# FAST-ASR/MarkovModels.jl

Measured on AMD Instinct MI355X. Metric: pdfposteriors_frames_per_sec, higher is better.
Workload: dtype f32

## Files before the change

markovmodels.jl_amd/csrc/mm_engine.hip:

```cpp
#include <hip/hip_runtime.h>
#include <dlfcn.h>

#include <algorithm>
#include <atomic>
#include <cmath>
#include <cstdio>
#include <cstdlib>
#include <chrono>
#include <cstring>
#include <limits>
#include <new>
#include <map>
#include <memory>
#include <mutex>
#include <string>
#include <thread>
#include <vector>

#include "../../include/markovmodels_amd.h"
#include "mm_kernels.hip"
#include "mm_kernel_quad.hip"
#include "mm_kernel_rows.hip"
#include "mm_internal.h"
#include "mm_pack.h"
// ... 851 lines not shown

static std::vector<float> init_by(mm_fsm_t f, const std::vector<int32_t> &order) {
    std::vector<float> v(size_t(f->S1));
    for (int64_t i = 0; i < f->S1; ++i) v[size_t(i)] = f->init[size_t(order[size_t(i)])];
    return v;
}

static int quad_variant(mm_fsm_t f, int dir, int KQ, bool verbose, QuadVariant **out) {
    auto it = f->variants.find(2 * KQ + dir);
    if (it != f->variants.end()) {
        *out = it->second.get();
        return MM_OK;
    }
    auto v = std::make_unique<QuadVariant>();
    v->KQ = KQ;
    v->dir = dir;
    v->g = make_quads(f->S1, f->qmat[dir].rowptr, f->qmat[dir].col, f->qmat[dir].val, f->s2p, f->P1, dir == 1, KQ);
    if (verbose)
        fprintf(stderr, "[mm] quad form dir %d: KQ %d, %zu quads, %lld arcs, LDS cycles/gather (bank model) %.2f -> %.2f\n",
                dir, KQ, v->g.quads.size(), (long long)f->qmat[dir].rowptr[f->S1], v->g.conflict_before,
                v->g.conflict_after);
    if (dir == 0) {
        v->init_f = init_by(f, v->g.order);
    } else {
        std::vector<int32_t> order_f, pos_f;
        quad_order(f->S1, f->qmat[0].rowptr, f->s2p, f->P1, false, order_f, pos_f);
        v->map_bf.resize(f->S1);
        for (int64_t i = 0; i < f->S1; ++i) v->map_bf[i] = uint16_t(pos_f[v->g.order[i]]);
    }
    {
        std::vector<int32_t> seeds;
        if (dir == 0) {
            for (int64_t s = 0; s < f->S1; ++s)
                if (f->init[s] > -std::numeric_limits<float>::infinity()) seeds.push_back(int32_t(s));
        } else {
            seeds.push_back(int32_t(f->S1 - 1));
        }
        const std::vector<uint16_t> d0 = reach_distance(f->S1, f->qmat[1 - dir].rowptr, f->qmat[1 - dir].col, seeds);
        v->dist.resize(f->S1);
        for (int64_t i = 0; i < f->S1; ++i) v->dist[i] = d0[v->g.order[i]];
    }
    Blob bl;
    const size_t o_q = bl.add(v->g.quads), o_rec = bl.add(v->g.recs), o_ptr = bl.add(v->g.rowptr);
    const size_t o_col = bl.add(v->g.col), o_w = bl.add(v->g.w), o_pse = bl.add(v->g.pdfstart);
    const size_t o_dist = bl.add(v->dist), o_initf = bl.add(v->init_f), o_map = bl.add(v->map_bf);
    int rc = upload(bl, v->blob);
    if (rc) return rc;
    char *base = static_cast<char *>(v->blob.get());
    v->qdev.quads = reinterpret_cast<const Quad *>(base + o_q);
    v->qdev.recs = reinterpret_cast<const RowRec *>(base + o_rec);
    v->qdev.rowptr = reinterpret_cast<const int *>(base + o_ptr);
    v->qdev.col = reinterpret_cast<const int *>(base + o_col);
    v->qdev.w = reinterpret_cast<const float *>(base + o_w);
    v->qdev.pdfse = reinterpret_cast<const unsigned short *>(base + o_pse);
    v->qdev.dist = reinterpret_cast<const unsigned short *>(base + o_dist);
    v->qdev.nq = int(v->g.quads.size());
    v->qdev.fpos = v->g.pos[f->S1 - 1];
    v->qdev.ncopy = v->g.ncopy;
    v->qdev.pad = 0;
    v->d_init_f = reinterpret_cast<const float *>(base + o_initf);
    v->d_map_bf = reinterpret_cast<const unsigned short *>(base + o_map);
    *out = v.get();
    f->variants[2 * KQ + dir] = std::move(v);
    return MM_OK;
}

struct RowBlob {
    Blob bl;
    size_t o_w, o_a, o_s, o_sc, o_ptr, o_col, o_cw, o_pdf, o_pse, o_init, o_ord, o_pt;
};
static void row_variant_blob(RowVariant &v, bool pad, RowBlob &rb) {
    if (pad) {
        v.g.w.resize(size_t(MM_ROW_KA_PAD) * 64 * v.g.NWC, 0.f);
        v.g.addr.resize(size_t(MM_ROW_KA_PAD) * 64 * v.g.NWC, 0u);
    }
    Blob &bl = rb.bl;
    rb.o_w = bl.add(v.g.w), rb.o_a = bl.add(v.g.addr), rb.o_s = bl.add(v.g.slots), rb.o_sc = bl.add(v.g.sched);
    rb.o_ptr = bl.add(v.g.rowptr), rb.o_col = bl.add(v.g.col), rb.o_cw = bl.add(v.g.cw);
    rb.o_pdf = bl.add(v.g.rowpdf), rb.o_pse = bl.add(v.g.pdfse), rb.o_init = bl.add(v.init), rb.o_ord = bl.add(v.g.order);
    rb.o_pt = bl.add(v.ptab);
}
static void row_variant_bind(mm_fsm_t f, RowVariant &v, const RowBlob &rb, char *base, float thr) {
    RowDev &d = v.rdev;
    d.w = reinterpret_cast<const float *>(base + rb.o_w);
    d.addr = reinterpret_cast<const unsigned *>(base + rb.o_a);
    d.slots = reinterpret_cast<const unsigned *>(base + rb.o_s);
    d.sched = reinterpret_cast<const RowSched *>(base + rb.o_sc);
    d.rowptr = reinterpret_cast<const int *>(base + rb.o_ptr);
    d.col = reinterpret_cast<const int *>(base + rb.o_col);
    d.cw = reinterpret_cast<const float *>(base + rb.o_cw);
    d.rowpdf = reinterpret_cast<const unsigned short *>(base + rb.o_pdf);
    d.pdfse = reinterpret_cast<const unsigned short *>(base + rb.o_pse);
    d.init = reinterpret_cast<const float *>(base + rb.o_init);
    d.order = reinterpret_cast<const int *>(base + rb.o_ord);
    d.ptab = v.ptab.empty() ? nullptr : reinterpret_cast<const unsigned *>(base + rb.o_pt);
    d.KA = v.g.KA;
    d.NWC = v.g.NWC;
    d.nslotrows = v.g.nslotrows;
    d.fpos = v.g.pos[f->S1 - 1];
    d.rows = int(f->S1);
    d.thr = thr;
}
static int upload_row_variant(mm_fsm_t f, RowVariant &v, float thr, bool pad = true) {
    RowBlob rb;
    row_variant_blob(v, pad, rb);
    DevMem mem;
    int rc = upload(rb.bl, mem);
    if (rc) return rc;
    v.mem = std::move(mem);
    row_variant_bind(f, v, rb, static_cast<char *>(v.mem.get()), thr);
    return MM_OK;
}


static RowPackOpts row_pack_opts(bool windows) {
    const size_t n = sizeof(kRowKA) / sizeof(kRowKA[0]);
    RowPackOpts opt;
    opt.rs = MM_ROW_RS;
    opt.ka_max = kRowKA[n - 1];
    for (size_t i = 0; i < n && windows; ++i) opt.ka_choices[i] = kRowKA[i];
    return opt;
}

static RowPackOpts pair_pack_opts(const DebugOpts &dbg, int dir, bool lag) {
    RowPackOpts opt;
    opt.rs = MM_ROW_RS;
    opt.ka_max = MM_PAIR_KA;
    opt.pair = true;
    opt.pdf_halves = !dbg.no_pdf_halves;
    for (float &x : opt.group_speed) x = 1.f;
    if (dbg.finish_cost > 0) opt.finish_cost = dbg.finish_cost;
    else if (dir == 1) opt.finish_cost = 24;
    if (dbg.group_speed[0] > 0) {
        for (int i = 0; i < 4; ++i) opt.group_speed[i] = dbg.group_speed[i];
    } else if (dir == 1 && lag) {
        const float sp[4] = {1.08f, 1.04f, 0.97f, 0.92f};
        for (int i = 0; i < 4; ++i) opt.group_speed[i] = sp[i];
    }
    opt.ka_choices[0] = MM_PAIR_KA;
    opt.bank_opt = dbg.bankopt ? 1 : 0;
    return opt;
}

static void split_pack_opts(const DebugOpts &dbg, RowPackOpts &opt, RowPackOpts &optb, int H = 2) {
    opt = RowPackOpts();
    opt.rs = mm_split_rs(H);
    opt.ka_max = mm_split_ka(H);
    opt.nwc_max = MM_SPLIT_NWC;
    opt.pair = true;
    opt.pdf_halves = !dbg.no_pdf_halves;
    for (float &x : opt.group_speed) x = 1.f;
    if (dbg.finish_cost > 0) opt.finish_cost = dbg.finish_cost;
    opt.ka_choices[0] = mm_split_ka(H);
    optb = opt;
    if (dbg.finish_cost <= 0) optb.finish_cost = 24;
}

static RowPackOpts wave_pack_opts(bool lean) {
    RowPackOpts opt;
    opt.rs = MM_WAVE_RS;
    opt.nwc_max = MM_WAVE_WAVES;
    opt.ka_max = 16;
    opt.copies = 1;
    opt.acap_force = 4;
    opt.seg_stride = 4;
    opt.log_weights = true;
    opt.want_partner = true;
    opt.spread_pdf = true;
    opt.finish_cost = 4;
    for (float &x : opt.group_speed) x = 1.f;
    if (!lean) return opt;
    opt.place = 1;
    opt.naive_stats = false;
    opt.q_positions = false;
    if (process_debug_opts().wave_place >= 0) opt.place = process_debug_opts().wave_place;
    return opt;
}

static RowPackOpts vit_pack_opts() {
    RowPackOpts opt;
    opt.rs = 65536;
    opt.nwc_max = 15;
    opt.copies = 1;
    opt.acap_force = 4;
    opt.log_weights = true;
    opt.keep_order = true;
    opt.finish_cost = 4;
    for (float &x : opt.group_speed) x = 1.f;
    return opt;
}


static RowForms pack_both(mm_fsm_t f, const RowPackOpts &opt, const RowPackOpts &optb, bool partner) {
    RowForms rv = std::make_unique<RowVariant[]>(2);
    const Csr *m = f->qmat;
    const std::vector<int32_t> none;
    if (!make_rows(f->S1, m[0].rowptr, m[0].col, m[0].val, f->s2p, f->P1, false, none, opt, rv[0].g) ||
        !make_rows(f->S1, m[1].rowptr, m[1].col, m[1].val, f->s2p, f->P1, true, rv[0].g.pos, optb, rv[1].g))
        return nullptr;
    if (partner) set_partner(rv[0].g, rv[1].g.pos);
    rv[0].init = init_by(f, rv[0].g.order);
    return rv;
}
static float wmin_log2(const RowForms &rv) { return std::min(rv[0].g.wmin_log2, rv[1].g.wmin_log2); }

static void say_rows(const char *name, int dir, const RowGraph &g) {
    fprintf(stderr, "[mm] %s form dir %d: KA %d, %d compute waves, %d segments, arcs/slots %.3f, cost %d..%d, "
                    "LDS cycles/gather (bank model) %.2f -> %.2f\n",
            name, dir, g.KA, g.NWC, g.nslotrows - 2, g.pad_eff, g.mincost, g.maxcost, g.conflict_before, g.conflict_after);
}

static int row_variants(mm_fsm_t f, bool verbose, bool *ok) {
    if (!f->rows.first(ok)) return MM_OK;
    if (f->semiring != MM_LOG || !f->fast_ok || f->P1 > 250 || (f->S1 + 1) * 4 > MM_ROW_RS) return MM_OK;
    RowForms rv = pack_both(f, row_pack_opts(true), row_pack_opts(true), false);
    if (!rv || !(wmin_log2(rv) >= -60.f)) return MM_OK;
    for (int dir = 0; dir < 2; ++dir) {
        const RowGraph &g = rv[dir].g;
        if (verbose) say_rows("row", dir, g);
        for (int w = 0; w < g.NWC && verbose; ++w) {
            const RowSched &sc = g.sched[w];
            int last = 0;
            for (int k = 0; k < 64; ++k)
                if ((sc.endmask >> k) & 1) last = k;
            fprintf(stderr, "[mm]   wave %2d: %u segments, %d arcs, lg %llx\n", w, sc.nslots & 0xffffu,
                    2 * (last + 1 - int(sc.nslots >> 16)), (unsigned long long)sc.lg);
        }
        int rc = upload_row_variant(f, rv[dir], 125.f + wmin_log2(rv));
        if (rc) return rc;
    }
    f->rows.form = std::move(rv);
    *ok = true;
    return MM_OK;
}

static int pair_variants(mm_fsm_t f, const DebugOpts &dbg, bool *ok) {
    const bool verbose = dbg.verbose;
    if (!f->prows.first(ok)) return MM_OK;
    if (f->semiring != MM_LOG || !f->fast_ok || f->P1 > MM_PAIR_P1MAX || (f->S1 + 1) * 4 > MM_ROW_RS) {
        if (verbose) fprintf(stderr, "[mm] pair form: not tried (semiring %d, fast_ok %d, P1 %d, S1 %lld)\n", f->semiring, int(f->fast_ok), int(f->P1), (long long)f->S1);
        return MM_OK;
    }
    RowForms rv = pack_both(f, pair_pack_opts(dbg, 0, true), pair_pack_opts(dbg, 1, true), true);
    if (verbose && !rv) fprintf(stderr, "[mm] pair form: the graph does not fit the register windows (KA %d)\n", MM_PAIR_KA);
    if (rv && wmin_log2(rv) < -60.f) {
        if (verbose) fprintf(stderr, "[mm] pair form: arc weights down to 2^%.0f\n", wmin_log2(rv));
        rv.reset();
    }
    if (!rv) return MM_OK;
    for (int dir = 0; dir < 2; ++dir) {
        if (verbose) say_rows("pair", dir, rv[dir].g);
        int rc = upload_row_variant(f, rv[dir], 125.f + wmin_log2(rv));
        if (rc) return rc;
    }
    f->prows.form = std::move(rv);
    *ok = true;
    return MM_OK;
}

static int vit_variant(mm_fsm_t f, const DebugOpts &dbg, bool *ok) {
    if (!f->vrow.first(ok)) return MM_OK;
    if (f->semiring != MM_TROPICAL || f->P1 > 256) return MM_OK;
    RowPackOpts opt = vit_pack_opts();
    RowForms rv = std::make_unique<RowVariant[]>(1);
    RowVariant &v = rv[0];
    const std::vector<int32_t> none;
    static const int shapes[3][2] = {{1, 5}, {2, 4}, {6, 0}};
    bool fits = false;
    for (const auto &sh : shapes) {
        opt.mix_n4 = sh[0];
        opt.mix_n2 = sh[1];
        opt.ka_max = 4 * sh[0] + 2 * sh[1];
        if (make_rows(f->S1, f->mat[0].rowptr, f->mat[0].col, f->mat[0].val, f->s2p, f->P1, false, none, opt, v.g)) {
            fits = true;
            f->vit_n4 = sh[0];
            f->vit_n2 = sh[1];
            break;
        }
    }
    if (!fits) return MM_OK;
    v.init = init_by(f, v.g.order);
    if (dbg.verbose)
        fprintf(stderr, "[mm] Viterbi form: %d waves, %d segments, %d x 4 + %d x 2 arc slots per lane, arcs/slots %.3f\n", v.g.NWC,
                v.g.nslotrows - 2, f->vit_n4, f->vit_n2, v.g.pad_eff);
    int rc = upload_row_variant(f, v, 0.f, false);
    if (rc) return rc;
    f->vrow.form = std::move(rv);
    *ok = true;
    return MM_OK;
}

static int lane_variant(mm_fsm_t f, bool *ok) {
    if (!f->lane.first(ok)) return MM_OK;
    const int64_t S = f->S1 - 1;
    const int P = f->P1 - 1;
    if (f->semiring != MM_LOG || S < 1 || S > 64 || P < 1 || P > 64) return MM_OK;
    for (int64_t s = 0; s < S; ++s)
        if (f->s2p[size_t(s)] >= P) return MM_OK;
    std::vector<double> w0(64 * 64, 0.0), w1(64 * 64, 0.0);
    std::vector<float> init(64, -std::numeric_limits<float>::infinity()), fin(64, -std::numeric_limits<float>::infinity());
    std::vector<int32_t> s2p(64, 0), pdf_ptr(size_t(P) + 1, 0), pdf_states(64, 0);
    const Csr &fwd = f->mat[0], &bwd = f->mat[1];
    for (int64_t j = 0; j < S; ++j)
        for (int64_t k = fwd.rowptr[size_t(j)]; k < fwd.rowptr[size_t(j) + 1]; ++k)
            if (fwd.col[size_t(k)] < S) w0[size_t(fwd.col[size_t(k)]) * 64 + size_t(j)] += std::exp2(double(fwd.val[size_t(k)]));
    for (int64_t i = 0; i < S; ++i)
// ... 2104 lines not shown
```

markovmodels.jl_amd/csrc/mm_rows.cpp:

```cpp
#include "mm_rows.h"
#include <cstdio>
#include <atomic>
#include <chrono>
#include <cstdlib>

#include <algorithm>
#include <cmath>
#include <cstdlib>
#include <cstring>
#include <limits>
#include <numeric>

namespace mm {
namespace {

struct Unit {
    int32_t row;
    int g;
    int A;
    int deg;
};
struct Segment {
    int g, A;
    std::vector<int32_t> rows;
    int wave = -1;
};

int log2i(int g) {
    int l = 0;
    while ((1 << l) < g) ++l;
    return l;
}

struct Banks {
    struct E {
        uint32_t addr;
        uint16_t n, bank;
    };
    E ent[64];
    int nent = 0, sqsum = 0;
    uint8_t cnt[32] = {0};
    static int of(uint32_t a) { return int(a >> 2) & 31; }
    int find(uint32_t a) const {
        for (int i = 0; i < nent; ++i)
            if (ent[i].addr == a) return i;
        return -1;
    }
    void add(uint32_t a) {
        const int i = find(a);
        if (i >= 0) {
            ++ent[i].n;
            return;
        }
        if (nent >= 64) std::abort();
        const int bk = of(a);
        ent[nent++] = E{a, 1, uint16_t(bk)};
        sqsum += 2 * cnt[bk] + 1;
        ++cnt[bk];
    }
    void remove(uint32_t a) {
        const int i = find(a);
        if (i < 0) return;
        if (--ent[i].n == 0) {
            const int bk = ent[i].bank;
            --cnt[bk];
            sqsum -= 2 * cnt[bk] + 1;
            ent[i] = ent[--nent];
        }
    }
    int cost_of(uint32_t a) const {
        return find(a) >= 0 ? 0 : int(cnt[of(a)]);
    }
    int cycles() const {
        int m = 1;
        for (int c : cnt) m = std::max(m, c);
        return m;
    }
    int sq() const { return sqsum; }
    bool conflicted(uint32_t a) const { return cnt[of(a)] > 1; }
    int least_loaded() const {
        int b = 0;
        for (int i = 1; i < 32; ++i)
            if (cnt[i] < cnt[b]) b = i;
        return b;
    }
};

struct Plan {
    std::vector<Segment> segs;
    std::vector<std::vector<int>> wave_segs;
    int KA = 0, maxcost = 0, mincost = 0;
    bool ok = false;
    std::vector<int> n4;
};

Plan plan_for(const std::vector<int32_t> &rows, const std::vector<int64_t> &rowptr, int acap, const RowPackOpts &opt,
              const std::vector<int32_t> *row2pdf = nullptr) {
    Plan p;
    std::vector<Unit> units;
    units.reserve(rows.size());
    for (int32_t r : rows) {
        const int d = int(rowptr[r + 1] - rowptr[r]);
        int g = 1;
        while ((std::max(d, 1) + g - 1) / g > acap / opt.a_round * opt.a_round && g < 64) g *= 2;
        int A = (std::max(d, 1) + g - 1) / g;
        A = (A + opt.a_round - 1) / opt.a_round * opt.a_round;
        units.push_back(Unit{int32_t(r), g, A, d});
    }
    for (int g = 1; g <= 64; g *= 2) {
        std::vector<Unit> us;
        for (auto &u : units)
            if (u.g == g) us.push_back(u);
        if (us.empty()) continue;
        std::stable_sort(us.begin(), us.end(), [](const Unit &a, const Unit &b) { return a.A > b.A; });
        const size_t per = size_t(64 / g);
        if (opt.spread_pdf && row2pdf) {
            for (size_t i0 = 0; i0 < us.size();) {
                size_t i1 = i0;
                while (i1 < us.size() && us[i1].A == us[i0].A) ++i1;
                const size_t n = i1 - i0, nseg = (n + per - 1) / per;
                if (nseg > 1) {
                    std::vector<Unit> run(us.begin() + i0, us.begin() + i1), out(n);
                    std::stable_sort(run.begin(), run.end(), [&](const Unit &a, const Unit &b) { return (*row2pdf)[a.row] < (*row2pdf)[b.row]; });
                    std::vector<size_t> fill(nseg, 0), cap(nseg, per);
                    cap[nseg - 1] = n - per * (nseg - 1);
                    size_t sgm = 0;
                    for (size_t j = 0; j < n; ++j) {
                        while (fill[sgm] >= cap[sgm]) sgm = (sgm + 1) % nseg;
                        out[sgm * per + fill[sgm]++] = run[j];
                        sgm = (sgm + 1) % nseg;
                    }
                    std::copy(out.begin(), out.end(), us.begin() + i0);
                }
                i0 = i1;
            }
        }
        for (size_t i = 0; i < us.size(); i += per) {
            Segment s;
            s.g = g;
            s.A = us[i].A;
            for (size_t j = i; j < std::min(us.size(), i + per); ++j) s.rows.push_back(us[j].row);
            p.segs.push_back(std::move(s));
        }
    }
    if (opt.pdf_halves && row2pdf) {
        long long before = 0, after = 0;
        auto half_cost = [&](const Segment &sg) {
            long long c = 0;
            const int per_half = 32 / std::min(sg.g, 32);
            for (int h = 0; h < 2 && sg.g <= 32; ++h) {
                int distinct[32] = {0};
                std::vector<int32_t> seen;
                for (int j = h * per_half; j < std::min<int>((h + 1) * per_half, int(sg.rows.size())); ++j) {
                    const int32_t pd = (*row2pdf)[size_t(sg.rows[size_t(j)])];
                    if (std::find(seen.begin(), seen.end(), pd) == seen.end()) {
                        seen.push_back(pd);
                        ++distinct[pd & 31];
                    }
                }
                int m = 1;
                for (int d : distinct) m = std::max(m, d);
                c += m - 1;
            }
            return c;
        };
        for (auto &sg : p.segs) {
            if (sg.g > 16 || sg.rows.size() < 3) continue;
            before += half_cost(sg);
            const int per_half = 32 / sg.g, n = int(sg.rows.size());
            const int cap0 = std::min(per_half, n), cap1 = n - cap0;
            if (cap1 <= 0) continue;
            std::vector<int32_t> rows = sg.rows;
            std::stable_sort(rows.begin(), rows.end(), [&](int32_t a, int32_t b) {
                const int32_t pa = (*row2pdf)[size_t(a)], pb = (*row2pdf)[size_t(b)];
                return (pa & 31) != (pb & 31) ? (pa & 31) < (pb & 31) : pa < pb;
            });
            std::vector<int32_t> half[2];
            int nb[2][32] = {{0}, {0}};
            for (size_t i0 = 0; i0 < rows.size();) {
                size_t i1 = i0;
                const int32_t pd = (*row2pdf)[size_t(rows[i0])];
                while (i1 < rows.size() && (*row2pdf)[size_t(rows[i1])] == pd) ++i1;
                const int bk = pd & 31, free0 = cap0 - int(half[0].size()), free1 = cap1 - int(half[1].size());
                int h = nb[0][bk] < nb[1][bk] ? 0 : (nb[1][bk] < nb[0][bk] ? 1 : (free0 >= free1 ? 0 : 1));
                if ((h ? free1 : free0) <= 0) h = 1 - h;
                for (size_t i = i0; i < i1; ++i) {
                    if (int(half[h].size()) >= (h ? cap1 : cap0)) h = 1 - h;
                    if (half[h].empty() || (*row2pdf)[size_t(half[h].back())] != pd) ++nb[h][bk];
                    half[h].push_back(rows[i]);
                }
                i0 = i1;
            }
            std::vector<int32_t> out = half[0];
            out.insert(out.end(), half[1].begin(), half[1].end());
            Segment trial = sg;
            trial.rows = out;
            if (half_cost(trial) <= half_cost(sg)) sg.rows = std::move(out);
            after += half_cost(sg);
        }
        if (getenv("MM_VERBOSE_PLAN")) fprintf(stderr, "[mm] pdf_halves: extra LDS cycles of the emission reads %lld -> %lld (%zu segments)\n", before, after, p.segs.size());
    }
    const int nwc = std::max(1, std::min<int>(opt.nwc_max, int(p.segs.size())));
    auto cost = [&](const Segment &s) { return s.A + opt.finish_cost + opt.group_cost * log2i(s.g); };
    std::vector<int> idx(p.segs.size());
    std::iota(idx.begin(), idx.end(), 0);
    std::stable_sort(idx.begin(), idx.end(), [&](int a, int b) { return cost(p.segs[a]) > cost(p.segs[b]); });
    std::vector<int> load(nwc, 0), arcs(nwc, 0), used4(nwc, 0), used2(nwc, 0);
    p.wave_segs.assign(nwc, {});
    p.n4.assign(nwc, 0);
    auto level = [&](int w, int extra) { return float(load[w] + extra) / opt.group_speed[std::min(w >> 2, 3)]; };
    for (int i : idx) {
        int best = -1;
        const int c = cost(p.segs[i]);
        for (int w = 0; w < nwc; ++w) {
            if (int(p.wave_segs[w].size()) >= MM_ROW_MAX_SLOTS) continue;
            if (opt.mix_n4 >= 0) {
                const bool narrow = p.segs[i].A <= 2 && used2[w] < opt.mix_n2;
                if (!narrow && used4[w] >= opt.mix_n4) continue;
            } else if (arcs[w] + std::max(p.segs[i].A, opt.seg_stride) > opt.ka_max) {
                continue;
            }
            if (best < 0 || level(w, c) < level(best, c) || (level(w, c) == level(best, c) && arcs[w] < arcs[best])) best = w;
        }
        if (best < 0) return p;
        p.segs[i].wave = best;
        p.wave_segs[best].push_back(i);
        load[best] += cost(p.segs[i]);
        arcs[best] += std::max(p.segs[i].A, opt.seg_stride);
        if (opt.mix_n4 >= 0) {
            if (p.segs[i].A <= 2 && used2[best] < opt.mix_n2) ++used2[best];
            else ++used4[best];
        }
    }
    for (auto &ws : p.wave_segs)
        std::stable_sort(ws.begin(), ws.end(), [&](int a, int b) { return p.segs[a].A > p.segs[b].A; });
    if (opt.mix_n4 >= 0)
        for (int w = 0; w < nwc; ++w) p.n4[w] = used4[w];
    p.KA = *std::max_element(arcs.begin(), arcs.end());
    p.maxcost = 0;
    p.mincost = 1 << 30;
    for (int w = 0; w < nwc; ++w) {
        p.maxcost = std::max(p.maxcost, int(level(w, 0) + 0.5f));
        p.mincost = std::min(p.mincost, int(level(w, 0) + 0.5f));
    }
    p.ok = p.KA <= opt.ka_max && p.KA <= 128;
    return p;
}

}

}
extern "C" {
std::atomic<long long> mm_rows_prof_ns[8];
}
namespace mm {
#define PROF_LAP(i)                                                                                                              \
    do {                                                                                                                         \
        const auto now_ = std::chrono::steady_clock::now();                                                                      \
        mm_rows_prof_ns[i] += std::chrono::duration_cast<std::chrono::nanoseconds>(now_ - prof_t_).count();                          \
        prof_t_ = now_;                                                                                                          \
    } while (0)

static void optimise_banks(const Plan &plan, const std::vector<int64_t> &rowptr, const std::vector<int32_t> &col, std::vector<int32_t> &pos,
                           std::vector<int32_t> &order) {
    const int nseg = int(plan.segs.size());
    const int NH = 2 * nseg;
    std::vector<int> cap(size_t(NH), 0);
    std::vector<std::vector<std::pair<int, int>>> mem(pos.size());
    std::vector<int> D(size_t(NH) * 32, 0);
    {
        std::vector<int> cnt(pos.size(), 0);
        std::vector<int32_t> touched;
        for (int si = 0; si < nseg; ++si) {
            const Segment &s = plan.segs[size_t(si)];
            for (int half = 0; half < 2; ++half) {
                const int h = 2 * si + half;
                cap[size_t(h)] = s.A;
                touched.clear();
                for (int l = 0; l < 32; ++l) {
                    const int lane = half * 32 + l, grp = lane / s.g, sub = lane % s.g;
                    if (grp >= int(s.rows.size())) continue;
                    const int32_t r = s.rows[size_t(grp)];
                    int n = 0;
                    for (int64_t a = rowptr[r] + sub; a < rowptr[r + 1] && n < s.A; a += s.g, ++n) {
                        if (cnt[size_t(col[a])]++ == 0) touched.push_back(col[a]);
                    }
                }
                for (int32_t c : touched) {
                    mem[size_t(c)].push_back({h, cnt[size_t(c)]});
                    D[size_t(h) * 32 + size_t(pos[size_t(c)] & 31)] += cnt[size_t(c)];
                    cnt[size_t(c)] = 0;
                }
            }
        }
    }
    std::vector<int> seg_of(pos.size(), -1), lane_of(pos.size(), 0);
    std::vector<int> W(size_t(nseg) * 4 * 16, 0);
    for (int si = 0; si < nseg; ++si) {
        const Segment &s = plan.segs[size_t(si)];
        for (size_t j = 0; j < s.rows.size(); ++j) {
            const int32_t r = s.rows[j];
            seg_of[size_t(r)] = si;
            lane_of[size_t(r)] = int(j) * s.g + s.g - 1;
            ++W[(size_t(si) * 4 + size_t(lane_of[size_t(r)] / 16)) * 16 + size_t(pos[size_t(r)] & 15)];
        }
    }
    constexpr long long WX = 4096, WW = 256;
    auto phi = [&](int h, int d) -> long long {
        const int x = d - cap[size_t(h)];
        return (x > 0 ? WX * x : 0) + (long long)d * d;
    };
    auto wcost = [&](int c) -> long long { return c > 1 ? WW * (c - 1) : 0; };
    long long excess = 0;
    for (int h = 0; h < NH; ++h)
        for (int b = 0; b < 32; ++b) excess += std::max(0, D[size_t(h) * 32 + b] - cap[size_t(h)]);
    if (getenv("MM_VERBOSE_PLAN")) fprintf(stderr, "[mm] bank_opt: excess before %lld\n", excess);
    std::vector<int> dd(size_t(NH), 0);
    std::vector<int> th;
    std::vector<int32_t> all;
    for (int si = 0; si < nseg; ++si)
        for (int32_t r : plan.segs[size_t(si)].rows) all.push_back(r);
    const int nall = int(all.size());
    for (int pass = 0; pass < 40 && excess > 0; ++pass) {
        bool improved = false;
        const bool wide = pass >= 6 && getenv("MM_BANKOPT_WIDE") != nullptr;
        if (pass >= 6 && !wide) break;
        {
            for (int i = 0; i < nall; ++i)
                for (int j = i + 1; j < nall; ++j) {
                    const int32_t r = all[size_t(i)], t = all[size_t(j)];
                    if (!wide && seg_of[size_t(r)] != seg_of[size_t(t)]) break;
                    const int b = pos[size_t(r)] & 31, b2 = pos[size_t(t)] & 31;
                    if (b == b2) continue;
                    if (wide) {
                        bool hot = false;
                        for (auto &m : mem[size_t(r)]) hot = hot || D[size_t(m.first) * 32 + b] > cap[size_t(m.first)];
                        if (!hot) break;
                    }
                    th.clear();
                    for (auto &m : mem[size_t(r)]) {
                        if (dd[size_t(m.first)] == 0) th.push_back(m.first);
                        dd[size_t(m.first)] -= m.second;
                    }
                    for (auto &m : mem[size_t(t)]) {
                        if (dd[size_t(m.first)] == 0) th.push_back(m.first);
                        dd[size_t(m.first)] += m.second;
                    }
                    long long delta = 0;
                    for (int h : th) {
                        const int d = dd[size_t(h)];
                        if (d == 0) continue;
                        const int o1 = D[size_t(h) * 32 + b], o2 = D[size_t(h) * 32 + b2];
                        delta += phi(h, o1 + d) - phi(h, o1) + phi(h, o2 - d) - phi(h, o2);
                    }
                    const int g1 = lane_of[size_t(r)] / 16, g2 = lane_of[size_t(t)] / 16;
                    const int c1 = pos[size_t(r)] & 15, c2 = pos[size_t(t)] & 15;
                    const int sr = seg_of[size_t(r)], st = seg_of[size_t(t)];
                    if ((g1 != g2 || sr != st) && c1 != c2) {
                        int *w1 = &W[(size_t(sr) * 4 + size_t(g1)) * 16], *w2 = &W[(size_t(st) * 4 + size_t(g2)) * 16];
                        delta += wcost(w1[c1] - 1) - wcost(w1[c1]) + wcost(w1[c2] + 1) - wcost(w1[c2]);
                        delta += wcost(w2[c2] - 1) - wcost(w2[c2]) + wcost(w2[c1] + 1) - wcost(w2[c1]);
                    }
                    if (delta < 0) {
                        for (int h : th) {
                            const int d = dd[size_t(h)];
                            if (d == 0) continue;
                            int &o1 = D[size_t(h) * 32 + b], &o2 = D[size_t(h) * 32 + b2];
                            excess -= std::max(0, o1 - cap[size_t(h)]) + std::max(0, o2 - cap[size_t(h)]);
                            o1 += d;
                            o2 -= d;
                            excess += std::max(0, o1 - cap[size_t(h)]) + std::max(0, o2 - cap[size_t(h)]);
                        }
                        if ((g1 != g2 || sr != st) && c1 != c2) {
                            int *w1 = &W[(size_t(sr) * 4 + size_t(g1)) * 16], *w2 = &W[(size_t(st) * 4 + size_t(g2)) * 16];
                            --w1[c1], ++w1[c2], --w2[c2], ++w2[c1];
                        }
                        std::swap(pos[size_t(r)], pos[size_t(t)]);
                        improved = true;
                    }
                    for (int h : th) dd[size_t(h)] = 0;
                }
        }
        if (!improved) break;
    }
    if (getenv("MM_VERBOSE_PLAN")) {
        long long tot = 0, slots = 0, mx = 0;
        for (int h = 0; h < NH; ++h) {
            int m = 0;
            for (int b = 0; b < 32; ++b) {
                tot += D[size_t(h) * 32 + b];
                m = std::max(m, D[size_t(h) * 32 + b] - cap[size_t(h)]);
            }
            mx += std::max(0, m);
            slots += 32ll * cap[size_t(h)];
        }
        fprintf(stderr, "[mm] bank_opt: %d half-segments, %lld arcs in %lld slots, excess %lld (sum over banks), %lld (sum of the half-segments' worst bank)\n", NH, tot, slots, excess, mx);
    }
    for (size_t r = 0; r < pos.size(); ++r)
        if (pos[r] >= 0) order[size_t(pos[r])] = int32_t(r);
}

static void colour_half_segment(int A, const std::vector<std::pair<int, int>> (&lane_arcs)[32], std::vector<int> (&slot_of)[32]) {
    struct Edge {
        int l, v, colour;
    };
    std::vector<Edge> ed;
    int bank_n[32] = {0};
    std::vector<std::pair<int, int>> where;
    for (int l = 0; l < 32; ++l) {
        slot_of[l].assign(lane_arcs[l].size(), -1);
        for (size_t i = 0; i < lane_arcs[l].size(); ++i) {
            const int b = lane_arcs[l][i].first;
            ed.push_back(Edge{l, b + 32 * (bank_n[b]++ / A), -1});
            where.push_back({l, int(i)});
        }
    }
    int nv = 32;
    for (auto &e : ed) nv = std::max(nv, e.v + 1);
    std::vector<int> lc(size_t(32) * A, -1), vc(size_t(nv) * A, -1);
    for (int e = 0; e < int(ed.size()); ++e) {
        const int l = ed[size_t(e)].l, v = ed[size_t(e)].v;
        int a = 0, b = 0;
        while (lc[size_t(l) * A + a] >= 0) ++a;
        while (vc[size_t(v) * A + b] >= 0) ++b;
        if (vc[size_t(v) * A + a] >= 0) {
            std::vector<int> path;
            int cur = vc[size_t(v) * A + a];
            bool want_b = true;
            while (cur >= 0) {
                path.push_back(cur);
                cur = want_b ? lc[size_t(ed[size_t(cur)].l) * A + b] : vc[size_t(ed[size_t(cur)].v) * A + a];
                want_b = !want_b;
            }
            for (int pe : path) {
                const Edge &x = ed[size_t(pe)];
                lc[size_t(x.l) * A + x.colour] = -1;
                vc[size_t(x.v) * A + x.colour] = -1;
            }
            for (int pe : path) {
                Edge &x = ed[size_t(pe)];
                x.colour = x.colour == a ? b : a;
                lc[size_t(x.l) * A + x.colour] = pe;
                vc[size_t(x.v) * A + x.colour] = pe;
            }
        }
        ed[size_t(e)].colour = a;
        lc[size_t(l) * A + a] = e;
        vc[size_t(v) * A + a] = e;
    }
    for (int e = 0; e < int(ed.size()); ++e) slot_of[where[size_t(e)].first][size_t(where[size_t(e)].second)] = ed[size_t(e)].colour;
}

bool make_rows(int64_t nrows, const std::vector<int64_t> &rowptr, const std::vector<int32_t> &col,
               const std::vector<float> &val, const std::vector<int32_t> &row2pdf, int32_t P1, bool backward,
               const std::vector<int32_t> &fwd_pos, const RowPackOpts &opt, RowGraph &g) {
    auto prof_t_ = std::chrono::steady_clock::now();
    g = RowGraph();
    std::vector<int32_t> myrows;
    if (opt.subset) {
        myrows = *opt.subset;
    } else {
        myrows.resize(size_t(nrows));
        std::iota(myrows.begin(), myrows.end(), 0);
    }
    const int64_t nsub = int64_t(myrows.size());
    const int64_t ntot = opt.gtrash >= 0 ? opt.gtrash : nrows;
    if (nrows < 1 || nsub < 1 || (ntot + 1) * (opt.pair ? 8 : 4) > (opt.pair ? 2 : 1) * opt.rs || (ntot + 1) * (opt.pair ? 8 : 4) > 65528 || P1 > 8000)
        return false;
    if (opt.copy_perm && ((ntot + 1 + 31) & ~int64_t(31)) * 4 > opt.rs) return false;
    Plan best;
    for (int acap : {4, 12, 16, 24, 32, 48, 64}) {
        if (opt.acap_force ? acap != opt.acap_force : (acap == 4 || acap > opt.ka_max)) continue;
        Plan p = plan_for(myrows, rowptr, acap, opt, &row2pdf);
        if (!p.ok && getenv("MM_VERBOSE_PLAN"))
            fprintf(stderr, "[mm] plan with at most %d arcs per lane and row: %zu segments on %zu waves, KA %d (limit %d)\n", acap, p.segs.size(),
                    p.wave_segs.size(), p.KA, opt.ka_max);
        if (!p.ok) continue;
        if (!best.ok || p.maxcost < best.maxcost || (p.maxcost == best.maxcost && p.KA < best.KA)) best = std::move(p);
    }
    if (!best.ok) return false;
    PROF_LAP(0);
    const int NWC = int(best.wave_segs.size());
    int KA = std::max(2, (best.KA + 1) & ~1);
    if (opt.mix_n4 >= 0) {
        KA = 4 * opt.mix_n4 + 2 * opt.mix_n2;
        for (auto &sg : best.segs)
            if (sg.A > 4) return false;
        if (opt.keep_order)
            for (int32_t r : myrows)
                if (rowptr[r + 1] - rowptr[r] > 255) return false;
    } else if (opt.seg_stride) {
        size_t most = 0;
        for (auto &ws : best.wave_segs) most = std::max(most, ws.size());
        KA = opt.seg_stride * int(most);
        if (KA > opt.ka_max) return false;
        for (auto &sg : best.segs)
            if (sg.A > opt.seg_stride) return false;
        if (opt.keep_order)
            for (int32_t r : myrows)
                if (rowptr[r + 1] - rowptr[r] > 255) return false;
    }
    for (int c : opt.ka_choices)
        if (c >= KA) {
            KA = c;
            break;
        }
    const int NT = 64 * NWC;
    g.KA = KA;
    g.NWC = NWC;
    g.rs = opt.rs;
    g.trash = int(ntot);
    g.pos_base = opt.pos_base;
    g.nrows = int(nsub);
    g.qtrash = int(nsub);
    g.slot_words = (backward || opt.pair || opt.want_partner) ? 2 : 1;
    g.scale = opt.pair ? 8 : 4;
    g.ncopy = opt.copies ? opt.copies : (opt.pair ? 1 : 2);
    const uint32_t SC = uint32_t(g.scale);
    const bool want_q = (backward || opt.pair || opt.want_partner) && opt.q_positions;
    g.maxcost = best.maxcost;
    g.mincost = best.mincost;
    g.order.assign(size_t(nsub), -1);
    g.pos.assign(size_t(nrows), -1);
    {
        int32_t next = 0;
        for (int w = 0; w < NWC; ++w)
            for (int si : best.wave_segs[w])
                for (int32_t r : best.segs[si].rows) {
                    g.pos[r] = next;
                    g.order[next] = r;
                    ++next;
                }
        if (next != nsub) return false;
    }
    const bool bank_opt = opt.bank_opt && opt.pair && !opt.subset && !opt.gpos && !opt.keep_order && opt.place >= 2 &&
                          (opt.copies ? opt.copies : 1) == 1 && !opt.log_weights && opt.mix_n4 < 0 && !opt.seg_stride;
    if (bank_opt) optimise_banks(best, rowptr, col, g.pos, g.order);
    if (opt.plan_only) return true;
    auto gp = [&](int32_t r) { return opt.gpos ? (*opt.gpos)[size_t(r)] : g.pos[size_t(r)]; };
    g.rowpdf.resize(size_t(nsub));
    for (int64_t i = 0; i < nsub; ++i) g.rowpdf[i] = uint16_t(row2pdf[g.order[i]]);
    std::vector<int32_t> qpos(size_t(nrows), 0);
    if (want_q) {
        std::vector<int32_t> byp(myrows);
        std::sort(byp.begin(), byp.end());
        std::stable_sort(byp.begin(), byp.end(), [&](int32_t a, int32_t b) { return row2pdf[a] < row2pdf[b]; });
        g.pdfse.assign(2 * size_t(P1), 0);
        std::vector<int64_t> first(P1, -1), last(P1, -1);
        for (int64_t i = 0; i < nsub; ++i) {
            qpos[byp[i]] = int32_t(i);
            const int32_t p = row2pdf[byp[i]];
            if (first[p] < 0) first[p] = i;
            last[p] = i;
        }
        for (int32_t p = 0; p < P1; ++p) {
            g.pdfse[2 * p] = uint16_t(first[p] < 0 ? 0 : first[p]);
            g.pdfse[2 * p + 1] = uint16_t(first[p] < 0 ? 0 : last[p] + 1);
        }
        std::vector<char> taken(size_t(nsub), 0);
        std::fill(qpos.begin(), qpos.end(), -1);
        const int G = opt.pair ? 16 : 32;
        const int trash_bank = int(nsub % 32);
        for (int w = 0; w < NWC; ++w)
            for (int si : best.wave_segs[w]) {
                const Segment &sg = best.segs[si];
                for (int l0 = 0; l0 < 64; l0 += G) {
                    unsigned used = (sg.g > 1 || int(sg.rows.size()) * sg.g < 64) ? 1u << trash_bank : 0u;
                    for (int l = l0; l < l0 + G; ++l) {
                        if (l % sg.g != sg.g - 1 || l / sg.g >= int(sg.rows.size())) continue;
                        const int32_t r = sg.rows[l / sg.g], pd = row2pdf[r];
                        int64_t pick = -1;
                        for (int64_t q = first[pd]; q <= last[pd]; ++q)
                            if (!taken[q]) {
                                if (pick < 0) pick = q;
                                if (!((used >> (q % 32)) & 1u)) {
                                    pick = q;
                                    break;
                                }
                            }
                        taken[pick] = 1;
                        used |= 1u << (pick % 32);
                        qpos[r] = int32_t(pick);
                    }
                }
            }
    }
    PROF_LAP(1);
    g.rowptr.assign(size_t(nsub) + 1, 0);
    g.col.clear();
    g.cw.clear();
    {
        int64_t a_out = 0;
        for (int64_t i = 0; i < nsub; ++i) {
            const int64_t r = g.order[i];
            g.rowptr[i] = int32_t(a_out);
            for (int64_t a = rowptr[r]; a < rowptr[r + 1]; ++a, ++a_out) {
                g.col.push_back(gp(col[a]));
                g.cw.push_back(val[a]);
            }
        }
        g.rowptr[nsub] = int32_t(a_out);
    }
    PROF_LAP(2);
    const int zero_pdf = (P1 + 3) & ~3;
    g.sched.assign(NWC, RowSched{0, 0, 0, 0});
    int nslots = 0;
    for (int w = 0; w < NWC; ++w) nslots += int(best.wave_segs[w].size());
    g.nslotrows = nslots + 2;
    g.slots.assign(size_t(g.nslotrows) * 64 * g.slot_words, 0);
    g.w.assign(size_t(KA) * NT, opt.log_weights ? -std::numeric_limits<float>::infinity() : 0.f);
    g.addr.assign(size_t(KA) * NT, 0u);
    const uint32_t copy1 = uint32_t(opt.copy_perm ? opt.rs : opt.rs + 64);
    const uint32_t ncopy = uint32_t(g.ncopy);
    const bool perm = opt.copy_perm;
    g.copy1 = (opt.pair ? 2u : 1u) * copy1;
    g.perm = perm;
    auto enc = [&](uint32_t c, uint32_t cp) { return cp ? copy1 + 4u * (perm ? (c ^ ((c >> 5) & 31u)) : c) : 4u * c; };
    auto other = [&](uint32_t a) {
        if (a >= copy1) {
            const uint32_t s = (a - copy1) / 4u;
            return 4u * (perm ? (s ^ ((s >> 5) & 31u)) : s);
        }
        return enc(a / 4u, 1);
    };
    double cyc_naive = 0, cyc_sched = 0;
    int64_t n_instr = 0, real_arcs = 0;
    int slotrow = 0;
    for (int w = 0; w < NWC; ++w) {
        RowSched &sc = g.sched[w];
        sc.slot0 = uint32_t(slotrow);
        int arcs_w = 0;
        for (int si : best.wave_segs[w]) arcs_w += best.segs[si].A;
        (void)arcs_w;
        int k0 = 0, sidx = 0;
        sc.nslots = uint32_t(best.wave_segs[w].size()) | (uint32_t(k0 / 2) << 16);
        if (opt.mix_n4 >= 0) sc.nslots = uint32_t(best.wave_segs[w].size()) | (uint32_t(best.n4[w]) << 16);
        for (int si : best.wave_segs[w]) {
            const Segment &s = best.segs[si];
            const int lg = log2i(s.g);
            if (opt.seg_stride) k0 = opt.seg_stride * sidx;
            if (opt.mix_n4 >= 0) k0 = sidx < best.n4[w] ? 4 * sidx : 4 * opt.mix_n4 + 2 * (sidx - best.n4[w]);
            sc.lg |= uint64_t(lg) << (4 * sidx);
            sc.endmask |= uint64_t(1) << ((k0 + s.A) / 2 - 1);
            for (int l = 0; l < 64; ++l) {
                const size_t e = (size_t(slotrow) * 64 + l) * g.slot_words;
                const int grp = l / s.g;
                if (grp < int(s.rows.size()) && l % s.g == s.g - 1) {
                    const int32_t r = s.rows[grp];
                    g.slots[e] = uint32_t(SC * (g.pos_base + g.pos[r])) | (uint32_t(SC * row2pdf[r]) << 16);
                    if (g.slot_words == 2)
                        g.slots[e + 1] = uint32_t((opt.pair ? 8 : 4) * (fwd_pos.empty() ? 0 : fwd_pos[r])) | (uint32_t(SC * qpos[r]) << 16);
                } else {
                    g.slots[e] = uint32_t(SC * g.trash) | (uint32_t(SC * zero_pdf) << 16);
                    if (g.slot_words == 2) g.slots[e + 1] = 0u | (uint32_t(SC * g.qtrash) << 16);
                }
            }
            for (int half = 0; half < 2; ++half) {
                static thread_local std::vector<Banks> tabn_s, tab_s;
                static thread_local std::vector<int64_t> la_s;
                static thread_local std::vector<uint32_t> ad_s;
                static thread_local std::vector<float> wt_s;
                static thread_local std::vector<char> used_s;
                if (tab_s.size() < size_t(s.A)) tab_s.resize(size_t(s.A));
                if (opt.naive_stats && tabn_s.size() < size_t(s.A)) tabn_s.resize(size_t(s.A));
                for (int k = 0; k < s.A; ++k) {
                    tab_s[size_t(k)] = Banks();
                    if (opt.naive_stats) tabn_s[size_t(k)] = Banks();
                }
                Banks *const tab = tab_s.data(), *const tabn = tabn_s.data();
                struct LaneArcs {
                    const int64_t *p;
                    size_t n;
// ... 339 lines not shown
```

markovmodels.jl_amd/csrc/mm_rows.h:

```cpp
#pragma once
#include <cstdint>
#include <vector>

namespace mm {

enum { MM_ROW_MAX_SLOTS = 16 };

struct RowSched {
    uint64_t endmask;
    uint64_t lg;
    uint32_t slot0;
    uint32_t nslots;
};
static_assert(sizeof(RowSched) == 24, "RowSched must be 24 bytes");

struct RowGraph {
    int KA = 0;
    int NWC = 0;
    int rs = 0;
    int nslotrows = 0;
    int trash = 0;
    int pos_base = 0;
    int nrows = 0;
    int qtrash = 0;
    std::vector<int32_t> order;
    std::vector<int32_t> pos;
    std::vector<float> w;
    std::vector<uint32_t> addr;
    std::vector<uint32_t> slots;
    int slot_words = 1;
    int scale = 4;
    int ncopy = 2;
    uint32_t copy1 = 0;
    bool perm = false;
    std::vector<RowSched> sched;
    std::vector<uint16_t> rowpdf;
    std::vector<int32_t> rowptr, col;
    std::vector<float> cw;
    std::vector<uint16_t> pdfse;
    double conflict_before = 0, conflict_after = 0;
    double pad_eff = 0;
    float wmin_log2 = 0;
    int maxcost = 0, mincost = 0;
};

struct RowPackOpts {
    int nwc_max = 15;
    int ka_max = 48;
    int rs = 8192;
    int finish_cost = 8;
    int group_cost = 2;
    float group_speed[4] = {1.0f, 0.92f, 0.80f, 0.70f};
    bool pair = false;
    int a_round = 2;
    int copies = 0;
    bool copy_perm = false;
    int ka_choices[8] = {0, 0, 0, 0, 0, 0, 0, 0};
    const std::vector<int32_t> *subset = nullptr;
    const std::vector<int32_t> *gpos = nullptr;
    int pos_base = 0;
    int gtrash = -1;
    bool plan_only = false;
    int acap_force = 0;
    int seg_stride = 0;
    bool log_weights = false;
    bool want_partner = false;
    bool spread_pdf = false;
    bool keep_order = false;
    int mix_n4 = -1, mix_n2 = 0;
    int place = 2;
    int bank_opt = 0;
    bool pdf_halves = false;
    bool naive_stats = true;
    bool q_positions = true;
};

bool make_rows(int64_t nrows, const std::vector<int64_t> &rowptr, const std::vector<int32_t> &col,
               const std::vector<float> &val_log2, const std::vector<int32_t> &row2pdf, int32_t P1, bool backward,
               const std::vector<int32_t> &fwd_pos, const RowPackOpts &opt, RowGraph &out);

struct SplitInfo {
    int H = 0;
    int total = 0;
    int base[8] = {0};
    int count[8] = {0};
    std::vector<int32_t> part;
    std::vector<int32_t> gpos[2];
};
bool make_rows_split(int H, int64_t nrows, const std::vector<int64_t> &fwd_ptr, const std::vector<int32_t> &fwd_col,
                     const std::vector<float> &fwd_val, const std::vector<int64_t> &bwd_ptr, const std::vector<int32_t> &bwd_col,
                     const std::vector<float> &bwd_val, const std::vector<int32_t> &row2pdf, int32_t P1, const RowPackOpts &opt_f,
                     const RowPackOpts &opt_b, std::vector<RowGraph> &out, SplitInfo &info);

void set_partner(RowGraph &g, const std::vector<int32_t> &partner_pos);

void eval_rows(const RowGraph &g, const float *in_lin, float *out_lin);

void eval_rows_log(const RowGraph &g, int seg_stride, const float *in_log2, float *out_log2);

}
```

Measured before the change: 140.9 million.

## Search every lane cap and swap segments between waves when packing rows

The host-side row packer now tries every even arcs-per-lane cap from 12 up to the KA limit, not a fixed short list. It skips caps that give the same lane grouping and prunes plans whose lower-bound load already exceeds the best cost found. When no wave has room for a segment, it can now move or swap an existing segment to another wave. The pdf-halves bank reordering runs once on the winning plan instead of on every candidate. The goal is a better-balanced per-wave schedule for the kernel, at the cost of more preprocessing time, and the split path turns the new search off.

```diff
diff --git a/markovmodels.jl_amd/csrc/mm_engine.hip b/markovmodels.jl_amd/csrc/mm_engine.hip
--- a/markovmodels.jl_amd/csrc/mm_engine.hip
+++ b/markovmodels.jl_amd/csrc/mm_engine.hip
@@ -1027,6 +1027,7 @@
     for (float &x : opt.group_speed) x = 1.f;
     if (dbg.finish_cost > 0) opt.finish_cost = dbg.finish_cost;
     opt.ka_choices[0] = mm_split_ka(H);
+    opt.every_cap = false;
     optb = opt;
     if (dbg.finish_cost <= 0) optb.finish_cost = 24;
 }
diff --git a/markovmodels.jl_amd/csrc/mm_rows.cpp b/markovmodels.jl_amd/csrc/mm_rows.cpp
--- a/markovmodels.jl_amd/csrc/mm_rows.cpp
+++ b/markovmodels.jl_amd/csrc/mm_rows.cpp
@@ -91,18 +91,119 @@
     std::vector<std::vector<int>> wave_segs;
     int KA = 0, maxcost = 0, mincost = 0;
     bool ok = false;
+    int exchanges = 0;
+    bool pruned = false;
     std::vector<int> n4;
 };
 
+void deal_pdf_halves(Plan &p, const std::vector<int32_t> &row2pdf) {
+    long long before = 0, after = 0;
+    auto half_cost = [&](const Segment &sg) {
+        long long c = 0;
+        const int per_half = 32 / std::min(sg.g, 32);
+        for (int h = 0; h < 2 && sg.g <= 32; ++h) {
+            int distinct[32] = {0};
+            std::vector<int32_t> seen;
+            for (int j = h * per_half; j < std::min<int>((h + 1) * per_half, int(sg.rows.size())); ++j) {
+                const int32_t pd = row2pdf[size_t(sg.rows[size_t(j)])];
+                if (std::find(seen.begin(), seen.end(), pd) == seen.end()) {
+                    seen.push_back(pd);
+                    ++distinct[pd & 31];
+                }
+            }
+            int m = 1;
+            for (int d : distinct) m = std::max(m, d);
+            c += m - 1;
+        }
+        return c;
+    };
+    for (auto &sg : p.segs) {
+        if (sg.g > 16 || sg.rows.size() < 3) continue;
+        before += half_cost(sg);
+        const int per_half = 32 / sg.g, n = int(sg.rows.size());
+        const int cap0 = std::min(per_half, n), cap1 = n - cap0;
+        if (cap1 <= 0) continue;
+        std::vector<int32_t> rows = sg.rows;
+        std::stable_sort(rows.begin(), rows.end(), [&](int32_t a, int32_t b) {
+            const int32_t pa = row2pdf[size_t(a)], pb = row2pdf[size_t(b)];
+            return (pa & 31) != (pb & 31) ? (pa & 31) < (pb & 31) : pa < pb;
+        });
+        std::vector<int32_t> half[2];
+        int nb[2][32] = {{0}, {0}};
+        for (size_t i0 = 0; i0 < rows.size();) {
+            size_t i1 = i0;
+            const int32_t pd = row2pdf[size_t(rows[i0])];
+            while (i1 < rows.size() && row2pdf[size_t(rows[i1])] == pd) ++i1;
+            const int bk = pd & 31, free0 = cap0 - int(half[0].size()), free1 = cap1 - int(half[1].size());
+            int h = nb[0][bk] < nb[1][bk] ? 0 : (nb[1][bk] < nb[0][bk] ? 1 : (free0 >= free1 ? 0 : 1));
+            if ((h ? free1 : free0) <= 0) h = 1 - h;
+            for (size_t i = i0; i < i1; ++i) {
+                if (int(half[h].size()) >= (h ? cap1 : cap0)) h = 1 - h;
+                if (half[h].empty() || row2pdf[size_t(half[h].back())] != pd) ++nb[h][bk];
+                half[h].push_back(rows[i]);
+            }
+            i0 = i1;
+        }
+        std::vector<int32_t> out = half[0];
+        out.insert(out.end(), half[1].begin(), half[1].end());
+        Segment trial = sg;
+        trial.rows = out;
+        if (half_cost(trial) <= half_cost(sg)) sg.rows = std::move(out);
+        after += half_cost(sg);
+    }
+    if (getenv("MM_VERBOSE_PLAN")) fprintf(stderr, "[mm] pdf_halves: extra LDS cycles of the emission reads %lld -> %lld (%zu segments)\n", before, after, p.segs.size());
+}
+
+int lanes_for(int d, int acap, const RowPackOpts &opt) {
+    int g = 1;
+    while ((std::max(d, 1) + g - 1) / g > acap / opt.a_round * opt.a_round && g < 64) g *= 2;
+    return g;
+}
+
+template <class Cost, class Level>
+int make_room(Plan &p, int A, int c, int ka_max, std::vector<int> &load, std::vector<int> &arcs, const Cost &cost, const Level &level) {
+    const int nwc = int(p.wave_segs.size());
+    int bw = -1, bw2 = -1, bj = -1, bk = -1;
+    float bl = 0.f;
+    for (int w = 0; w < nwc; ++w) {
+        if (int(p.wave_segs[w].size()) >= MM_ROW_MAX_SLOTS) continue;
+        for (int j = 0; j < int(p.wave_segs[w].size()); ++j) {
+            const Segment &sj = p.segs[p.wave_segs[w][j]];
+            for (int w2 = 0; w2 < nwc; ++w2) {
+                if (w2 == w) continue;
+                for (int k = -1; k < int(p.wave_segs[w2].size()); ++k) {
+                    if (k < 0 && int(p.wave_segs[w2].size()) >= MM_ROW_MAX_SLOTS) continue;
+                    const int Ak = k < 0 ? 0 : p.segs[p.wave_segs[w2][k]].A, ck = k < 0 ? 0 : cost(p.segs[p.wave_segs[w2][k]]);
+                    if (Ak >= sj.A || arcs[w] - sj.A + Ak + A > ka_max || arcs[w2] - Ak + sj.A > ka_max) continue;
+                    const float l = std::max(level(w, c + ck - cost(sj)), level(w2, cost(sj) - ck));
+                    if (bw < 0 || l < bl) bw = w, bw2 = w2, bj = j, bk = k, bl = l;
+                }
+            }
+        }
+    }
+    if (bw < 0) return -1;
+    const int sj = p.wave_segs[bw][bj], sk = bk < 0 ? -1 : p.wave_segs[bw2][bk];
+    if (sk < 0) {
+        p.wave_segs[bw].erase(p.wave_segs[bw].begin() + bj);
+        p.wave_segs[bw2].push_back(sj);
+    } else {
+        std::swap(p.wave_segs[bw][bj], p.wave_segs[bw2][bk]);
+        p.segs[sk].wave = bw;
+    }
+    p.segs[sj].wave = bw2;
+    const int dA = p.segs[sj].A - (sk < 0 ? 0 : p.segs[sk].A), dc = cost(p.segs[sj]) - (sk < 0 ? 0 : cost(p.segs[sk]));
+    arcs[bw] -= dA, arcs[bw2] += dA, load[bw] -= dc, load[bw2] += dc;
+    return bw;
+}
+
 Plan plan_for(const std::vector<int32_t> &rows, const std::vector<int64_t> &rowptr, int acap, const RowPackOpts &opt,
-              const std::vector<int32_t> *row2pdf = nullptr) {
+              const std::vector<int32_t> *row2pdf = nullptr, int bound = std::numeric_limits<int>::max()) {
     Plan p;
     std::vector<Unit> units;
     units.reserve(rows.size());
     for (int32_t r : rows) {
         const int d = int(rowptr[r + 1] - rowptr[r]);
-        int g = 1;
-        while ((std::max(d, 1) + g - 1) / g > acap / opt.a_round * opt.a_round && g < 64) g *= 2;
+        const int g = lanes_for(d, acap, opt);
         int A = (std::max(d, 1) + g - 1) / g;
         A = (A + opt.a_round - 1) / opt.a_round * opt.a_round;
         units.push_back(Unit{int32_t(r), g, A, d});
@@ -143,63 +244,6 @@
             p.segs.push_back(std::move(s));
         }
     }
-    if (opt.pdf_halves && row2pdf) {
-        long long before = 0, after = 0;
-        auto half_cost = [&](const Segment &sg) {
-            long long c = 0;
-            const int per_half = 32 / std::min(sg.g, 32);
-            for (int h = 0; h < 2 && sg.g <= 32; ++h) {
-                int distinct[32] = {0};
-                std::vector<int32_t> seen;
-                for (int j = h * per_half; j < std::min<int>((h + 1) * per_half, int(sg.rows.size())); ++j) {
-                    const int32_t pd = (*row2pdf)[size_t(sg.rows[size_t(j)])];
-                    if (std::find(seen.begin(), seen.end(), pd) == seen.end()) {
-                        seen.push_back(pd);
-                        ++distinct[pd & 31];
-                    }
-                }
-                int m = 1;
-                for (int d : distinct) m = std::max(m, d);
-                c += m - 1;
-            }
-            return c;
-        };
-        for (auto &sg : p.segs) {
-            if (sg.g > 16 || sg.rows.size() < 3) continue;
-            before += half_cost(sg);
-            const int per_half = 32 / sg.g, n = int(sg.rows.size());
-            const int cap0 = std::min(per_half, n), cap1 = n - cap0;
-            if (cap1 <= 0) continue;
-            std::vector<int32_t> rows = sg.rows;
-            std::stable_sort(rows.begin(), rows.end(), [&](int32_t a, int32_t b) {
-                const int32_t pa = (*row2pdf)[size_t(a)], pb = (*row2pdf)[size_t(b)];
-                return (pa & 31) != (pb & 31) ? (pa & 31) < (pb & 31) : pa < pb;
-            });
-            std::vector<int32_t> half[2];
-            int nb[2][32] = {{0}, {0}};
-            for (size_t i0 = 0; i0 < rows.size();) {
-                size_t i1 = i0;
-                const int32_t pd = (*row2pdf)[size_t(rows[i0])];
-                while (i1 < rows.size() && (*row2pdf)[size_t(rows[i1])] == pd) ++i1;
-                const int bk = pd & 31, free0 = cap0 - int(half[0].size()), free1 = cap1 - int(half[1].size());
-                int h = nb[0][bk] < nb[1][bk] ? 0 : (nb[1][bk] < nb[0][bk] ? 1 : (free0 >= free1 ? 0 : 1));
-                if ((h ? free1 : free0) <= 0) h = 1 - h;
-                for (size_t i = i0; i < i1; ++i) {
-                    if (int(half[h].size()) >= (h ? cap1 : cap0)) h = 1 - h;
-                    if (half[h].empty() || (*row2pdf)[size_t(half[h].back())] != pd) ++nb[h][bk];
-                    half[h].push_back(rows[i]);
-                }
-                i0 = i1;
-            }
-            std::vector<int32_t> out = half[0];
-            out.insert(out.end(), half[1].begin(), half[1].end());
-            Segment trial = sg;
-            trial.rows = out;
-            if (half_cost(trial) <= half_cost(sg)) sg.rows = std::move(out);
-            after += half_cost(sg);
-        }
-        if (getenv("MM_VERBOSE_PLAN")) fprintf(stderr, "[mm] pdf_halves: extra LDS cycles of the emission reads %lld -> %lld (%zu segments)\n", before, after, p.segs.size());
-    }
     const int nwc = std::max(1, std::min<int>(opt.nwc_max, int(p.segs.size())));
     auto cost = [&](const Segment &s) { return s.A + opt.finish_cost + opt.group_cost * log2i(s.g); };
     std::vector<int> idx(p.segs.size());
@@ -209,6 +253,17 @@
     p.wave_segs.assign(nwc, {});
     p.n4.assign(nwc, 0);
     auto level = [&](int w, int extra) { return float(load[w] + extra) / opt.group_speed[std::min(w >> 2, 3)]; };
+    {
+        float total = 0.f, speed = 0.f, fastest = 0.f;
+        for (int w = 0; w < nwc; ++w) speed += opt.group_speed[std::min(w >> 2, 3)], fastest = std::max(fastest, opt.group_speed[std::min(w >> 2, 3)]);
+        for (const Segment &sg : p.segs) total += float(cost(sg));
+        const float lb = std::max(total / speed, idx.empty() ? 0.f : float(cost(p.segs[idx[0]])) / fastest);
+        if (int(lb + 0.5f) > bound) {
+            p.pruned = true;
+            return p;
+        }
+    }
+    const bool may_exchange = opt.every_cap && opt.mix_n4 < 0 && !opt.seg_stride && !opt.acap_force;
     for (int i : idx) {
         int best = -1;
         const int c = cost(p.segs[i]);
@@ -221,6 +276,10 @@
                 continue;
             }
             if (best < 0 || level(w, c) < level(best, c) || (level(w, c) == level(best, c) && arcs[w] < arcs[best])) best = w;
+        }
+        if (best < 0 && may_exchange) {
+            best = make_room(p, p.segs[i].A, c, opt.ka_max, load, arcs, cost, level);
+            p.exchanges += best >= 0;
         }
         if (best < 0) return p;
         p.segs[i].wave = best;
@@ -468,17 +527,45 @@
     if (nrows < 1 || nsub < 1 || (ntot + 1) * (opt.pair ? 8 : 4) > (opt.pair ? 2 : 1) * opt.rs || (ntot + 1) * (opt.pair ? 8 : 4) > 65528 || P1 > 8000)
         return false;
     if (opt.copy_perm && ((ntot + 1 + 31) & ~int64_t(31)) * 4 > opt.rs) return false;
+    std::vector<int> degs;
+    for (int32_t r : myrows) degs.push_back(int(rowptr[r + 1] - rowptr[r]));
+    std::sort(degs.begin(), degs.end());
+    degs.erase(std::unique(degs.begin(), degs.end()), degs.end());
+    std::vector<int> caps;
+    const int cap_top = std::min(opt.ka_max, 64);
+    if (opt.acap_force) {
+        caps.push_back(opt.acap_force);
+    } else if (opt.every_cap) {
+        for (int c = 12; c <= cap_top; c += 2) caps.push_back(c);
+    } else {
+        for (int c : {12, 16, 24, 32, 48, 64})
+            if (c <= cap_top) caps.push_back(c);
+    }
+    std::vector<int> lanes, lanes_before;
     Plan best;
-    for (int acap : {4, 12, 16, 24, 32, 48, 64}) {
-        if (opt.acap_force ? acap != opt.acap_force : (acap == 4 || acap > opt.ka_max)) continue;
-        Plan p = plan_for(myrows, rowptr, acap, opt, &row2pdf);
-        if (!p.ok && getenv("MM_VERBOSE_PLAN"))
-            fprintf(stderr, "[mm] plan with at most %d arcs per lane and row: %zu segments on %zu waves, KA %d (limit %d)\n", acap, p.segs.size(),
-                    p.wave_segs.size(), p.KA, opt.ka_max);
+    for (int acap : caps) {
+        lanes.clear();
+        for (int d : degs) lanes.push_back(lanes_for(d, acap, opt));
+        if (lanes == lanes_before) continue;
+        lanes_before = lanes;
+        Plan p = plan_for(myrows, rowptr, acap, opt, &row2pdf, best.ok ? best.maxcost : std::numeric_limits<int>::max());
+        if (!p.ok && getenv("MM_VERBOSE_PLAN")) {
+            if (p.pruned)
+                fprintf(stderr, "[mm] plan with at most %d arcs per lane and row: %zu segments, not dealt (its mean load is above the best cost %d)\n", acap,
+                        p.segs.size(), best.maxcost);
+            else
+                fprintf(stderr, "[mm] plan with at most %d arcs per lane and row: %zu segments on %zu waves, no wave has room for all (limit %d)\n", acap,
+                        p.segs.size(), p.wave_segs.size(), opt.ka_max);
+        }
         if (!p.ok) continue;
-        if (!best.ok || p.maxcost < best.maxcost || (p.maxcost == best.maxcost && p.KA < best.KA)) best = std::move(p);
+        if (getenv("MM_VERBOSE_PLAN"))
+            fprintf(stderr, "[mm] plan with at most %d arcs per lane and row: %zu segments, cost %d..%d, KA %d\n", acap, p.segs.size(), p.mincost, p.maxcost, p.KA);
+        if (!best.ok || p.maxcost < best.maxcost || (p.maxcost == best.maxcost && p.KA < best.KA) ||
+            (opt.every_cap && p.maxcost == best.maxcost && p.KA == best.KA && p.segs.size() < best.segs.size()))
+            best = std::move(p);
     }
     if (!best.ok) return false;
+    if (opt.pdf_halves) deal_pdf_halves(best, row2pdf);
     PROF_LAP(0);
     const int NWC = int(best.wave_segs.size());
     int KA = std::max(2, (best.KA + 1) & ~1);
@@ -518,6 +605,7 @@
     g.ncopy = opt.copies ? opt.copies : (opt.pair ? 1 : 2);
     const uint32_t SC = uint32_t(g.scale);
     const bool want_q = (backward || opt.pair || opt.want_partner) && opt.q_positions;
+    g.exchanges = best.exchanges;
     g.maxcost = best.maxcost;
     g.mincost = best.mincost;
     g.order.assign(size_t(nsub), -1);
diff --git a/markovmodels.jl_amd/csrc/mm_rows.h b/markovmodels.jl_amd/csrc/mm_rows.h
--- a/markovmodels.jl_amd/csrc/mm_rows.h
+++ b/markovmodels.jl_amd/csrc/mm_rows.h
@@ -42,6 +42,7 @@
     double pad_eff = 0;
     float wmin_log2 = 0;
     int maxcost = 0, mincost = 0;
+    int exchanges = 0;
 };
 
 struct RowPackOpts {
@@ -71,6 +72,7 @@
     int place = 2;
     int bank_opt = 0;
     bool pdf_halves = false;
+    bool every_cap = true;
     bool naive_stats = true;
     bool q_positions = true;
 };
```

Result: faster. 146.3 million (median of 6 runs) (+3.8%).
